# MMOCKING/RIDERS

Measured on AMD Instinct MI355X. Metric: train imgs/sec (RC-Net+SML, 256x512), higher is better.
Workload: dtype bf16; 1 GPU; 2 RC-Net steps (batch 8, K=30, patch 240x100, 256x512) + 1 SML step (batch 16, 256x512) per iteration = 16 images through BOTH stages; each step fwd+loss+bwd+Adam; global_batch=16, parallelism=dp1

## Files before the change

riders_amd/csrc/rd_api.cpp:

```cpp
#include "../../include/riders_hip.h"
#include "rd_kernels.h"
#define rd rd_f16
#include "rd_kernels_decl.h"
#undef rd
#include <math.h>
#include <stdarg.h>
#include <stdio.h>
#include <string.h>
#include <stdlib.h>
#define RD_SLAB_DECL(NS) namespace NS { \
  bool bn_slab_ok(int64_t pixels, int C, int dtype); \
  void launch_bn_bwd_slab(const void* dz, const void* y, const float* mean, const float* rstd, const float* scale, const float* shift, float* dgamma, float* dbeta, \
                          int accumulate, void* dy, int64_t pixels, int C, int act, float slope, int dtype, hipStream_t st); \
  void launch_bn_fwd_slab(const float* stats, int rows, const void* y, const float* gamma, const float* beta, float eps, float momentum, float* running_mean, \
                          float* running_var, float* mean, float* rstd, float* scale, float* shift, void* out, int64_t pixels, int C, int act, float slope, int dtype, \
                          hipStream_t st); \
  const char* bn_slab_kernel_name(int which, int64_t pixels, int dtype, int act); }
RD_SLAB_DECL(rd)
RD_SLAB_DECL(rd_f16)
#undef RD_SLAB_DECL
namespace rd { void launch_augment_vflip_boxes(float* boxes, int B, int K, const float* params, float n_height, hipStream_t st); }
namespace rd { void launch_pack_weights_batch_map(const void* items, int n, const void* map, int blocks, hipStream_t st); }
namespace rd_f16 { void launch_pack_weights_batch_map(const void* items, int n, const void* map, int blocks, hipStream_t st); }

// ... 31 lines not shown
  a.N = d->N; a.Hin = d->Hin; a.Win = d->Win; a.C1 = d->C1; a.C2 = d->C2;
  a.ups = d->upsample ? 1 : 0;
  a.H1 = a.ups ? d->H1 : d->Hin; a.W1 = a.ups ? d->W1 : d->Win;
  a.Cout = d->Cout; a.KH = d->KH; a.KW = d->KW; a.stride = d->stride; a.pad = d->pad; a.dil = d->in_dilate;
  a.OH = d->OH; a.OW = d->OW; a.act = d->act; a.slope = d->slope; a.D1 = d->D1;
  a.scale_h = (float)a.H1 / (float)d->Hin; a.scale_w = (float)a.W1 / (float)d->Win;
  a.M = d->N * d->OH * d->OW;
  a.K = d->KH * d->KW * (d->C1 + d->C2);
  a.Kpad = RD_NS(d->dtype, conv_kpad)(a.K, RD_DT(d->dtype));
  a.pool2 = d->out_reduce2 ? 1 : 0;
  a.d2s = d->out_d2s ? 1 : 0;
  a.s2d = d->in_s2d ? 1 : 0;
}
}

namespace {
struct OptDef { const char* name; int lo, hi; };
const OptDef kOpts[rdt::OPT_COUNT] = {
  {"conv_par", 0, 1}, {"conv3x3_min_blocks", 0, 1 << 30}, {"conv_stem_min_m", 0, 1 << 30}, {"wgrad_blocks", 8, 1 << 16}, {"wgrad_tiny_min_m", 0, 1 << 30},
  {"conv3x3_w8", 0, 1}, {"patch_bn_max", 32, 128}, {"conv3x3_g8", 1, 4096}, {"conv1x1_min_m", 0, 1 << 30}, {"conv_few_min_m", 0, 1 << 30},
  {"frag_v128", 0, 6}, {"frag_v64", 0, 6}, {"frag_v32", 0, 6}, {"frag_split", 0, 1}, {"frag_split_blocks", 0, 1 << 30},
  {"frag32_v128", 0, 3}, {"frag32_v64", 0, 3}, {"frag_lin", 0, 1}, {"conv3x3_frag", 0, 1}, {"bn_gen_ppt", 2, 64}, {"bn_vec_per", 0, 64},
  {"wgrad_tr_tw", 8, 32}, {"frag_db", 0, 1}, {"wgrad_fit", 0, 1}, {"head_np", 256, 1800}, {"head_cpi", 0, 0x888}, {"pw_min_m", 0, 1 << 30}, {"pw_ks", 0, 8}, {"bn_slab", 0, 2},
};
int g_opt_val[rdt::OPT_COUNT];
bool g_opt_set[rdt::OPT_COUNT];
}

extern "C" {

int rd_opt(int id, int dflt) { return (id >= 0 && id < rdt::OPT_COUNT && g_opt_set[id]) ? g_opt_val[id] : dflt; }
int rd_opt_is_set(int id) { return id >= 0 && id < rdt::OPT_COUNT && g_opt_set[id]; }
int rd_set_option(const char* name, int32_t value) {
  if (!name) return fail("set_option: null name");
  for (int i = 0; i < rdt::OPT_COUNT; i++)
    if (!strcmp(name, kOpts[i].name)) {
      g_opt_val[i] = value < kOpts[i].lo ? kOpts[i].lo : (value > kOpts[i].hi ? kOpts[i].hi : value);
      g_opt_set[i] = true;
      return 0;
    }
  return fail("set_option: unknown option '%s'", name);
}
int rd_clear_options(void) { for (int i = 0; i < rdt::OPT_COUNT; i++) g_opt_set[i] = false; return 0; }
int rd_clear_option(const char* name) {
  if (!name) return rd_clear_options();
  for (int i = 0; i < rdt::OPT_COUNT; i++) if (!strcmp(name, kOpts[i].name)) { g_opt_set[i] = false; return 0; }
// ... 999 lines not shown
```

riders_amd/csrc/rd_dwconv.hip:

```cpp
#include "rd_common.h"
#include "rd_kernels.h"

namespace rd {

static unsigned ew_grid(int64_t n) { return (unsigned)std::max<int64_t>(1, std::min<int64_t>(cdiv(n, 256), 4096)); }

template <typename T>
__global__ __launch_bounds__(256) void dwconv_fwd_kernel(const T* __restrict__ x, const float* __restrict__ w, T* __restrict__ y,
                                                         int N, int H, int W, int C, int OH, int OW, int k, int s, int p) {
  const int64_t total = (int64_t)N * OH * OW * C;
  for (int64_t i = (int64_t)blockIdx.x * blockDim.x + threadIdx.x; i < total; i += (int64_t)gridDim.x * blockDim.x) {
    int c = (int)(i % C); int64_t q = i / C;
    int ow = (int)(q % OW); q /= OW; int oh = (int)(q % OH); int n = (int)(q / OH);
    float acc = 0.f;
    for (int kh = 0; kh < k; kh++) {
      int ih = oh * s - p + kh;
      if ((unsigned)ih >= (unsigned)H) continue;
      for (int kw = 0; kw < k; kw++) {
        int iw = ow * s - p + kw;
        if ((unsigned)iw >= (unsigned)W) continue;
        acc += Elem<T>::ld(x + (((int64_t)n * H + ih) * W + iw) * C + c) * w[(c * k + kh) * k + kw];
      }
    }
    Elem<T>::st(y + i, acc);
// ... 50 lines not shown
          acc[j] += g * Elem<T>::ld(x + (((int64_t)n * H + ih) * W + iw) * C + c);
      }
    }
  }
  for (int j = 0; j < k * k; j++) {
    float v = 0.f;
#pragma unroll
    for (int jj = 0; jj < KK; jj++) if (jj == j) v = acc[jj];
    red[t] = v;
    __syncthreads();
    if (pl == 0 && c < C) {
      float sacc = 0.f;
      for (int q = 0; q < PL; q++) sacc += red[q * CB + cl];
      partial[((int64_t)blockIdx.x * C + c) * (k * k) + j] = sacc;
    }
    __syncthreads();
  }
}


#ifndef RD_DW_ST_MODE
#define RD_DW_ST_MODE 1
#endif
static constexpr int DWR = 4;

static constexpr int DW_QMAX = 64;
template <int K> struct DwLds { static constexpr int STR = K == 5 ? 108 : 4 * K * K; };
template <int K>
__device__ __forceinline__ void dw_stage_weights(const float* __restrict__ w, int c0, int nq, float* lds, int cl, bool active,
                                                 float (&wr)[K * K][4]) {
  constexpr int QF = 4 * K * K, STR = DwLds<K>::STR;
  const float* src = w + (int64_t)c0 * K * K;
  if ((reinterpret_cast<uintptr_t>(src) & 15) == 0) {
    for (int i = threadIdx.x; i < nq * (QF / 4); i += blockDim.x) {
      const float4 v = reinterpret_cast<const float4*>(src)[i];
      const int qd = (i * 4) / QF, off = i * 4 - qd * QF;
      *reinterpret_cast<float4*>(lds + qd * STR + off) = v;
    }
  } else {
    for (int i = threadIdx.x; i < nq * QF; i += blockDim.x) { const int qd = i / QF; lds[qd * STR + i - qd * QF] = src[i]; }
  }
  __syncthreads();
  if (active) {
#pragma unroll
    for (int j = 0; j < K * K; j++)
#pragma unroll
      for (int e = 0; e < 4; e++) wr[j][e] = lds[cl * STR + e * K * K + j];
  }
}

template <typename T, int K, int S, int MODE, bool ST>
__global__ __launch_bounds__(256) RD_WAVES_PER_EU((ST && S == 1) ? 2 : 1) void dw_run_kernel(const T* __restrict__ src, const float* __restrict__ w, T* __restrict__ dst, int N,
                                                     int H, int W, int C, int OH, int OW, int p, int QB, int PL, int PPB,
                                                     float* __restrict__ stats) {
  __shared__ __attribute__((aligned(16))) float wl[DW_QMAX * DwLds<K>::STR];
  const int t = threadIdx.x, pl = t / QB, cl = t - pl * QB;
  const int c = (blockIdx.y * QB + cl) * 4;
  const bool active = pl < PL && c < C;
  float wr[K * K][4];
  dw_stage_weights<K>(w, blockIdx.y * QB * 4, min(QB, C / 4 - (int)blockIdx.y * QB), wl, cl, active, wr);
  if (!ST && !active) return;
  float* red = wl;
  if (ST) {
    __syncthreads();
#pragma unroll
    for (int e = 0; e < 8; e++) red[t * 8 + e] = 0.f;
  }
  constexpr int WIN = (DWR - 1) * S + K;
  const int DH = MODE ? H : OH, DW = MODE ? W : OW;
  const int SH = MODE ? OH : H, SW = MODE ? OW : W;
  const int runs = (DW + DWR - 1) / DWR;
  const int64_t M = (int64_t)N * DH * runs;
// ... 39 lines not shown
#pragma unroll
      for (int r = 0; r < DWR; r++)
        if (dw0 + r < DW) {
#pragma unroll
          for (int e = 0; e < 4; e++) { const float v = Elem<T>::rnd(acc[r][e]); u1[e] += v; u2[e] += v * v; }
        }
#pragma unroll
      for (int e = 0; e < 4; e++) { red[t * 8 + e] += u1[e]; red[t * 8 + 4 + e] += u2[e]; }
    }
  }
  if (ST) {
    __syncthreads();
#if RD_DW_ST_MODE == 0
    if (active && pl == 0) {
#pragma unroll
      for (int e = 0; e < 4; e++) {
        float a = 0.f, b = 0.f;
        for (int q = 0; q < PL; q++) { a += red[(q * QB + cl) * 8 + e]; b += red[(q * QB + cl) * 8 + 4 + e]; }
        stats[((int64_t)blockIdx.x * C + c + e) * 2] = a;
        stats[((int64_t)blockIdx.x * C + c + e) * 2 + 1] = b;
      }
    }
#elif RD_DW_ST_MODE == 1
    if (active) {
      for (int e8 = pl; e8 < 8; e8 += PL) {
        float a = 0.f;
        for (int q0 = 0; q0 < PL; q0 += 4) {
          float v[4];
#pragma unroll
          for (int u = 0; u < 4; u++) v[u] = red[(min(q0 + u, PL - 1) * QB + cl) * 8 + e8];
#pragma unroll
          for (int u = 0; u < 4; u++) if (q0 + u < PL) a += v[u];
        }
        stats[((int64_t)blockIdx.x * C + c + (e8 & 3)) * 2 + (e8 >> 2)] = a;
      }
    }
#else
    if (active && pl == 0 && red[t * 8] == 12345.f) stats[0] = 1.f;
#endif
  }
}

template <typename T, int K, int PP, int PH>
__device__ __forceinline__ void dw_dgrad2_rows(const T* __restrict__ dy, const float (&wr)[K * K][4], int n, int dh, int p, int OH, int OW, int C,
                                               int c, const int* coff, const bool* cok, float (&acc)[DWR][4]) {
  constexpr int NJ = (K + 2 - PP) / 2 + 1;
#pragma unroll
  for (int kh = PH; kh < K; kh += 2) {
    const int oh = (dh + p - kh) >> 1;
    const bool rok = (unsigned)oh < (unsigned)OH;
    const T* row = dy + (((int64_t)n * OH + (oh < 0 ? 0 : (oh >= OH ? OH - 1 : oh))) * OW) * C + c;
    float v[NJ][4];
#pragma unroll
    for (int j = 0; j < NJ; j++) ld4z(row + coff[j], rok && cok[j], v[j]);
#pragma unroll
    for (int r = 0; r < DWR; r++)
#pragma unroll
      for (int j = 0; j < NJ; j++) {
        const int kw = r + (K - 1 - PP) - 2 * j;
// ... 72 lines not shown
#pragma unroll
      for (int j = 0; j < WIN; j++) {
        const int iw = cbase + j;
        cok[j] = (unsigned)iw < (unsigned)W;
        coff[j] = (iw < 0 ? 0 : (iw >= W ? W - 1 : iw)) * C;
      }
#pragma unroll
      for (int kh = 0; kh < K; kh++) {
        const int ih = oh * S - p + kh;
        const bool rok = (unsigned)ih < (unsigned)H;
        const T* row = x + (((int64_t)n * H + (ih < 0 ? 0 : (ih >= H ? H - 1 : ih))) * W) * C + c;
        float v[WIN][4];
#pragma unroll
        for (int j = 0; j < WIN; j++) ld4z(row + coff[j], rok && cok[j], v[j]);
#pragma unroll
        for (int kw = 0; kw < K; kw++)
#pragma unroll
          for (int r = 0; r < DWR; r++)
#pragma unroll
            for (int e = 0; e < 4; e++) acc[kh * K + kw][e] = fmaf(g[r][e], v[r * S + kw][e], acc[kh * K + kw][e]);
      }
    }
  }
#pragma unroll
  for (int kh = 0; kh < K; kh++) {
#pragma unroll
    for (int kw = 0; kw < K; kw++)
#pragma unroll
      for (int e = 0; e < 4; e++) red[t][kw][e] = acc[kh * K + kw][e];
    __syncthreads();
    if (cv) {
      for (int kw = pl; kw < K; kw += PL) {
        float s4[4] = {0.f, 0.f, 0.f, 0.f};
        for (int q0 = 0; q0 < PL; q0 += 4) {
          float4 v[4];
#pragma unroll
          for (int u = 0; u < 4; u++) v[u] = *reinterpret_cast<const float4*>(&red[min(q0 + u, PL - 1) * QB + cl][kw][0]);
#pragma unroll
          for (int u = 0; u < 4; u++)
            if (q0 + u < PL) { s4[0] += v[u].x; s4[1] += v[u].y; s4[2] += v[u].z; s4[3] += v[u].w; }
        }
        st4(partial + ((int64_t)blockIdx.x * (K * K) + kh * K + kw) * C + c, s4);
      }
    }
    __syncthreads();
  }
}

__global__ __launch_bounds__(256) void dw_wgrad_finalize_tc_kernel(const float* __restrict__ partial, int rows, int C, int KK, float* dw,
                                                                   int accumulate) {
  __shared__ double red[4][64];
  const int e = threadIdx.x & 63, rg = threadIdx.x >> 6;
  const int i = blockIdx.x * 64 + e, CK = C * KK;
  double a = 0.0;
  if (i < CK)
    for (int r = rg; r < rows; r += 4) a += partial[(int64_t)r * CK + i];
  red[rg][e] = a;
  __syncthreads();
  if (rg == 0 && i < CK) {
    a = red[0][e] + red[1][e] + red[2][e] + red[3][e];
    const int j = i / C, c = i - j * C;
    const int o = c * KK + j;
    dw[o] = accumulate ? dw[o] + (float)a : (float)a;
  }
}

__global__ __launch_bounds__(64) void dwconv_wgrad_finalize_kernel(const float* __restrict__ partial, int rows, int CK, float* dw,
                                                                   int accumulate) {
  const int i = blockIdx.x, lane = threadIdx.x;
// ... 93 lines not shown
  for (int64_t i = (int64_t)blockIdx.x * blockDim.x + threadIdx.x; i < n; i += (int64_t)gridDim.x * blockDim.x) {
    float sc = 1.f + Elem<T>::ld(out + i);
    float p = d[i] * (sc > 0.f ? sc : 0.f);
    bool clamped = (hi > 0.f && p > hi);
    if (!clamped && lo > 0.f && p < lo) clamped = true;
    Elem<T>::st(dout + i, (sc > 0.f && !clamped) ? dpred[i] * d[i] : 0.f);
  }
}
__global__ __launch_bounds__(256) void reciprocal_kernel(const float* __restrict__ x, const float* __restrict__ dy, float* __restrict__ out,
                                                         int64_t n) {
  for (int64_t i = (int64_t)blockIdx.x * blockDim.x + threadIdx.x; i < n; i += (int64_t)gridDim.x * blockDim.x) {
    float v = x[i];
    out[i] = dy ? -dy[i] / (v * v) : 1.f / v;
  }
}

struct RG { int CB, PL, nchunk; };
static RG rgeom(int C) { RG g; int cb = 1; while (cb < C && cb < 256) cb <<= 1; g.CB = cb; g.PL = 256 / cb; g.nchunk = (int)cdiv(C, cb); return g; }
int dw_rows(int64_t pixels, int C) {
  RG g = rgeom(C);
  return (int)std::max<int64_t>(1, std::min<int64_t>(cdiv(pixels, (int64_t)g.PL * 64), 512));
}

struct QG { int QB, PL, nchunk; };
static QG qgeom(int C, int qmax) {
  const int c4 = C / 4;
  QG best = {1, 256, c4}; double bu = -1.0;
  for (int nc = 1; nc <= 256; nc++) {
    const int qb = (int)cdiv(c4, nc);
    if (qb > qmax) continue;
    const int pl = 256 / qb;
    const double u = (double)c4 * pl / (256.0 * nc);
    if (u > bu + 1e-9) { bu = u; best = {qb, pl, nc}; }
  }
  return best;
}
static int dw_upt(int64_t units, const QG& g) {
  (void)units; (void)g;
  return 1;
}
static int dw_stats_ppb(int64_t units, const QG& g) {
  const int64_t upt = std::max<int64_t>(dw_upt(units, g), cdiv(units, (int64_t)g.PL * 1024));
  return (int)(g.PL * upt);
}
template <typename T, int MODE>
static void launch_dw_quad(const void* src, const float* w, void* dst, int N, int H, int W, int C, int OH, int OW, int k, int s, int p, hipStream_t st,
                           float* stats = nullptr) {
  const QG g = qgeom(C, DW_QMAX);
  const int DH = MODE ? H : OH, DW = MODE ? W : OW;
  const int64_t units = (int64_t)N * DH * cdiv(DW, DWR);
  const int ppb = stats ? dw_stats_ppb(units, g) : g.PL * dw_upt(units, g);
  const dim3 grid((unsigned)cdiv(units, ppb), g.nchunk);
#define RD_DWQ(KERNEL) hipLaunchKernelGGL(KERNEL, grid, dim3(256), 0, st, (const T*)src, w, (T*)dst, N, H, W, C, OH, OW, p, g.QB, g.PL, ppb, stats)
#define RD_DWQ2(KERNEL) hipLaunchKernelGGL(KERNEL, grid, dim3(256), 0, st, (const T*)src, w, (T*)dst, N, H, W, C, OH, OW, p, g.QB, g.PL, ppb)
  if (MODE == 0 && stats) {
    if (s == 1) { if (k == 3) RD_DWQ((dw_run_kernel<T, 3, 1, 0, true>)); else RD_DWQ((dw_run_kernel<T, 5, 1, 0, true>)); }
    else { if (k == 3) RD_DWQ((dw_run_kernel<T, 3, 2, 0, true>)); else RD_DWQ((dw_run_kernel<T, 5, 2, 0, true>)); }
  } else if (MODE == 0) {
    if (s == 1) { if (k == 3) RD_DWQ((dw_run_kernel<T, 3, 1, 0, false>)); else RD_DWQ((dw_run_kernel<T, 5, 1, 0, false>)); }
    else { if (k == 3) RD_DWQ((dw_run_kernel<T, 3, 2, 0, false>)); else RD_DWQ((dw_run_kernel<T, 5, 2, 0, false>)); }
  } else if (s == 1) {
    if (k == 3) RD_DWQ((dw_run_kernel<T, 3, 1, 1, false>)); else RD_DWQ((dw_run_kernel<T, 5, 1, 1, false>));
  } else if (p & 1) {
    if (k == 3) RD_DWQ2((dw_dgrad2_kernel<T, 3, 1>)); else RD_DWQ2((dw_dgrad2_kernel<T, 5, 1>));
  } else {
    if (k == 3) RD_DWQ2((dw_dgrad2_kernel<T, 3, 0>)); else RD_DWQ2((dw_dgrad2_kernel<T, 5, 0>));
  }
#undef RD_DWQ
#undef RD_DWQ2
}
static bool dw_quad_ok(int C, int k, int s) { return C % 4 == 0 && (k == 3 || k == 5) && (s == 1 || s == 2); }

int dwconv_stats_rows(int N, int OH, int OW, int C, int k, int s) {
  if (!dw_quad_ok(C, k, s)) return 0;
  const QG g = qgeom(C, DW_QMAX);
  const int64_t units = (int64_t)N * OH * cdiv(OW, DWR);
  return (int)cdiv(units, dw_stats_ppb(units, g));
}
void launch_dwconv_fwd(const void* x, const float* w, void* y, int N, int H, int W, int C, int OH, int OW, int k, int s, int p, int dtype,
                       hipStream_t st, float* stats) {
  if (dw_quad_ok(C, k, s)) {
    if (dtype == 0) launch_dw_quad<float, 0>(x, w, y, N, H, W, C, OH, OW, k, s, p, st, stats);
    else launch_dw_quad<bf16_t, 0>(x, w, y, N, H, W, C, OH, OW, k, s, p, st, stats);
    return;
  }
  int64_t n = (int64_t)N * OH * OW * C;
  if (dtype == 0) hipLaunchKernelGGL((dwconv_fwd_kernel<float>), dim3(ew_grid(n)), dim3(256), 0, st, (const float*)x, w, (float*)y, N, H, W, C, OH, OW, k, s, p);
  else hipLaunchKernelGGL((dwconv_fwd_kernel<bf16_t>), dim3(ew_grid(n)), dim3(256), 0, st, (const bf16_t*)x, w, (bf16_t*)y, N, H, W, C, OH, OW, k, s, p);
}
void launch_dwconv_dgrad(const void* dy, const float* w, void* dx, int N, int H, int W, int C, int OH, int OW, int k, int s, int p,
                         int dtype, hipStream_t st) {
  if (dw_quad_ok(C, k, s)) {
    if (dtype == 0) launch_dw_quad<float, 1>(dy, w, dx, N, H, W, C, OH, OW, k, s, p, st);
    else launch_dw_quad<bf16_t, 1>(dy, w, dx, N, H, W, C, OH, OW, k, s, p, st);
    return;
  }
  int64_t n = (int64_t)N * H * W * C;
  if (dtype == 0) hipLaunchKernelGGL((dwconv_dgrad_kernel<float>), dim3(ew_grid(n)), dim3(256), 0, st, (const float*)dy, w, (float*)dx, N, H, W, C, OH, OW, k, s, p);
  else hipLaunchKernelGGL((dwconv_dgrad_kernel<bf16_t>), dim3(ew_grid(n)), dim3(256), 0, st, (const bf16_t*)dy, w, (bf16_t*)dx, N, H, W, C, OH, OW, k, s, p);
}
struct DwWgradBatch { DwWgradItem it[DW_WGRAD_BATCH_MAX]; };
__global__ __launch_bounds__(256) void dw_wgrad_finalize_batch_kernel(DwWgradBatch b) {
  __shared__ double red[4][64];
  const DwWgradItem it = b.it[blockIdx.y];
  const int e = threadIdx.x & 63, rg = threadIdx.x >> 6;
  const int CK = it.C * it.KK;
  for (int base = blockIdx.x * 64; base < CK; base += gridDim.x * 64) {
    const int i = base + e;
    double a = 0.0;
    if (i < CK) {
      for (int r = rg; r < it.rows; r += 32) {
        float v[8];
#pragma unroll
        for (int q = 0; q < 8; q++) { const int rq = r + 4 * q; const float x = it.partial[(int64_t)(rq < it.rows ? rq : 0) * CK + i]; v[q] = rq < it.rows ? x : 0.f; }
#pragma unroll
// ... 6 lines not shown
      a = red[0][e] + red[1][e] + red[2][e] + red[3][e];
      const int j = i / it.C, c = i - j * it.C;
      const int o = c * it.KK + j;
      it.dw[o] = it.accumulate ? it.dw[o] + (float)a : (float)a;
    }
    __syncthreads();
  }
}
void launch_dw_wgrad_finalize_batch(const DwWgradItem* items, int n, hipStream_t st) {
  for (int base = 0; base < n; base += DW_WGRAD_BATCH_MAX) {
    const int m = std::min(DW_WGRAD_BATCH_MAX, n - base);
    DwWgradBatch b;
    int maxg = 1;
    for (int i = 0; i < m; i++) { b.it[i] = items[base + i]; maxg = std::max(maxg, (int)cdiv(b.it[i].C * b.it[i].KK, 64)); }
    for (int i = m; i < DW_WGRAD_BATCH_MAX; i++) b.it[i] = b.it[0];
    hipLaunchKernelGGL(dw_wgrad_finalize_batch_kernel, dim3((unsigned)std::min(maxg, 1024), (unsigned)m), dim3(256), 0, st, b);
  }
}
void launch_dwconv_wgrad(const void* x, const void* dy, float* partial, float* dw, int accumulate, int N, int H, int W, int C, int OH,
                         int OW, int k, int s, int p, int dtype, hipStream_t st, DwWgradItem* item) {
  if (item) { item->partial = partial; item->dw = dw; item->rows = 0; item->C = C; item->KK = k * k; item->accumulate = accumulate; }
  const int rows = dw_rows((int64_t)N * OH * OW, C);
  if (dw_quad_ok(C, k, s)) {
    const QG g = qgeom(C, 256);
    const int64_t units = (int64_t)N * OH * cdiv(OW, DWR);
    int64_t gx = std::min<int64_t>(512 / g.nchunk, cdiv(units, (int64_t)g.PL * 3));
    gx = std::min<int64_t>(gx, std::max<int64_t>(64, (int64_t)N * OH * OW / 32));
    gx = std::max<int64_t>(1, std::min<int64_t>(gx, rows));
    const dim3 grid((unsigned)gx, g.nchunk);
#define RD_DWG(T, K, S) hipLaunchKernelGGL((dw_wgrad_run_kernel<T, K, S>), grid, dim3(256), 0, st, (const T*)x, (const T*)dy, partial, N, H, W, C, OH, OW, p, g.QB, g.PL)
    if (dtype == 0) {
      if (s == 1) { if (k == 3) RD_DWG(float, 3, 1); else RD_DWG(float, 5, 1); }
      else { if (k == 3) RD_DWG(float, 3, 2); else RD_DWG(float, 5, 2); }
    } else {
      if (s == 1) { if (k == 3) RD_DWG(bf16_t, 3, 1); else RD_DWG(bf16_t, 5, 1); }
      else { if (k == 3) RD_DWG(bf16_t, 3, 2); else RD_DWG(bf16_t, 5, 2); }
    }
#undef RD_DWG
    if (item) { item->rows = (int)gx; return; }
    hipLaunchKernelGGL(dw_wgrad_finalize_tc_kernel, dim3((unsigned)cdiv(C * k * k, 64)), dim3(256), 0, st, partial, (int)gx, C, k * k, dw, accumulate);
    return;
  }
  RG g = rgeom(C);
  dim3 grid(rows, g.nchunk);
#define RD_DW(T, KK) hipLaunchKernelGGL((dwconv_wgrad_kernel<T, KK>), grid, dim3(256), 0, st, (const T*)x, (const T*)dy, partial, N, H, W, C, OH, OW, k, s, p, g.CB, g.PL)
  if (dtype == 0) { if (k <= 3) RD_DW(float, 9); else RD_DW(float, 25); }
  else { if (k <= 3) RD_DW(bf16_t, 9); else RD_DW(bf16_t, 25); }
#undef RD_DW
  hipLaunchKernelGGL(dwconv_wgrad_finalize_kernel, dim3(C * k * k), dim3(64), 0, st, partial, rows, C * k * k, dw, accumulate);
}
void launch_bn_stats(const void* y, float* partial, int64_t pixels, int C, int dtype, hipStream_t st) {
  RG g = rgeom(C);
  dim3 grid(dw_rows(pixels, C), g.nchunk);
  if (dtype == 0) hipLaunchKernelGGL((bn_stats_kernel<float>), grid, dim3(256), 0, st, (const float*)y, partial, pixels, C, g.CB, g.PL);
  else hipLaunchKernelGGL((bn_stats_kernel<bf16_t>), grid, dim3(256), 0, st, (const bf16_t*)y, partial, pixels, C, g.CB, g.PL);
}
template <typename T>
__global__ __launch_bounds__(256) void bilinear_fwd_vec_kernel(const T* __restrict__ x, T* __restrict__ y, int N, int H, int W, int C, int OH,
                                                               int OW, int align) {
  constexpr int VE = Elem<T>::VE;
  const int CV = C / VE;
// ... 126 lines not shown
```

riders_amd/csrc/rd_types.h:

```cpp
#pragma once
#include <hip/hip_runtime.h>
#include <stdint.h>

namespace rdt {

struct ConvArgs {
  const void* src1; const void* src2; const void* w; const float* bias;
  void* dst1; void* dst2; float* stats;
  int N, Hin, Win, C1, C2, H1, W1, Cout, KH, KW, stride, pad, dil, OH, OW, act, D1;
  float slope, scale_h, scale_w;
  int M, K, Kpad, ups;
  int s2d;
  int d2s;
  int pool2;
  const void* add1;
  const float* in_scale; const float* in_shift; int in_act; float in_slope;
  const void* bn_y; const float *bn_scale, *bn_shift, *bn_mean, *bn_rstd; int bn_act; float bn_slope;
};

struct WgradArgs {
  const void* src1; const void* src2; const void* dy; float* slab;
  int N, Hin, Win, C1, C2, H1, W1, Cout, KH, KW, stride, pad, OH, OW;
  float scale_h, scale_w;
  int M, K, ups, nsplit, rows_per_split;
// ... 10 lines not shown

struct LnGradItem { const float* partial[4]; float* dgamma; float* dbeta; int rows[4]; int C, nparts, accumulate, reserved; };
static const int LN_GRAD_BATCH_MAX = 32;
struct DwWgradItem { const float* partial; float* dw; int rows, C, KK, accumulate; };
static const int DW_WGRAD_BATCH_MAX = 64;
struct ColsumItem { const float* partial; float* out; int rows, C, accumulate, reserved; };
static const int COLSUM_BATCH_MAX = 64;

static const int LWG_MAX_ITEMS = 64, LWG_MAX_REDS = 96;

struct LoftrW { const void *wq, *wk, *wv, *wm, *w0, *w2; const float *g1, *b1, *g2, *b2; };

struct LoftrSaved { void *q, *k, *v, *att, *mpre, *msg, *hid, *m2pre; float* stats; };

struct LoftrGrads {
  const void* dout; void *dm2pre, *dhid, *dmpre, *datt, *dq, *dk, *dv, *dx, *dsrc;
  float *lnp1, *lnp2, *dg1, *db1, *dg2, *db2; int accumulate, defer_ln;
  int dsrc_accumulate, reserved;
};

enum RdOpt {
  OPT_CONV_PAR, OPT_CONV3X3_MIN_BLOCKS, OPT_CONV_STEM_MIN_M, OPT_WGRAD_BLOCKS, OPT_WGRAD_TINY_MIN_M, OPT_CONV3X3_W8, OPT_PATCH_BN_MAX,
  OPT_CONV3X3_G8, OPT_CONV1X1_MIN_M, OPT_CONV_FEW_MIN_M, OPT_FRAG_V128, OPT_FRAG_V64, OPT_FRAG_V32, OPT_FRAG_SPLIT, OPT_FRAG_SPLIT_BLOCKS,
  OPT_FRAG32_V128, OPT_FRAG32_V64, OPT_FRAG_LIN, OPT_CONV3X3_FRAG, OPT_BN_GEN_PPT, OPT_BN_VEC_PER, OPT_WGRAD_TR_TW, OPT_FRAG_DB, OPT_WGRAD_FIT, OPT_HEAD_NP, OPT_HEAD_CPI, OPT_PW_MIN_M, OPT_PW_KS, OPT_BN_SLAB, OPT_COUNT
};

}

extern "C" int rd_opt(int id, int dflt);
extern "C" int rd_opt_is_set(int id);
```

Before: 618.6 imgs/s.

## Add column-strip depthwise conv kernels with rolling row window reuse

Adds new depthwise conv kernels where each thread walks down a strip of R output rows over a CW-wide column run. A rolling register window of input rows is reused across all K kernel rows, and the next row is prefetched while the current one is computed. The default mode (dw_col=1) routes forward and dgrad for stride-1 3x3/5x5 convs through the new path when the launch gives enough blocks. Weight-gradient and stats-fused variants are only used in mode 2. The aim is to cut redundant input loads versus the per-row quad kernel, at the cost of higher register pressure and fewer parallel work units.

```diff
diff --git a/riders_amd/csrc/rd_api.cpp b/riders_amd/csrc/rd_api.cpp
--- a/riders_amd/csrc/rd_api.cpp
+++ b/riders_amd/csrc/rd_api.cpp
@@ -77,6 +77,7 @@
   {"frag_v128", 0, 6}, {"frag_v64", 0, 6}, {"frag_v32", 0, 6}, {"frag_split", 0, 1}, {"frag_split_blocks", 0, 1 << 30},
   {"frag32_v128", 0, 3}, {"frag32_v64", 0, 3}, {"frag_lin", 0, 1}, {"conv3x3_frag", 0, 1}, {"bn_gen_ppt", 2, 64}, {"bn_vec_per", 0, 64},
   {"wgrad_tr_tw", 8, 32}, {"frag_db", 0, 1}, {"wgrad_fit", 0, 1}, {"head_np", 256, 1800}, {"head_cpi", 0, 0x888}, {"pw_min_m", 0, 1 << 30}, {"pw_ks", 0, 8}, {"bn_slab", 0, 2},
+  {"dw_col", 0, 2}, {"dw_col_rows", 0, 1024},
 };
 int g_opt_val[rdt::OPT_COUNT];
 bool g_opt_set[rdt::OPT_COUNT];
diff --git a/riders_amd/csrc/rd_dwconv.hip b/riders_amd/csrc/rd_dwconv.hip
--- a/riders_amd/csrc/rd_dwconv.hip
+++ b/riders_amd/csrc/rd_dwconv.hip
@@ -1,5 +1,4 @@
-#include "rd_common.h"
-#include "rd_kernels.h"
+#include "rd_dwconv_common.h"
 
 namespace rd {
 
@@ -96,32 +95,6 @@
 #ifndef RD_DW_ST_MODE
 #define RD_DW_ST_MODE 1
 #endif
-static constexpr int DWR = 4;
-
-static constexpr int DW_QMAX = 64;
-template <int K> struct DwLds { static constexpr int STR = K == 5 ? 108 : 4 * K * K; };
-template <int K>
-__device__ __forceinline__ void dw_stage_weights(const float* __restrict__ w, int c0, int nq, float* lds, int cl, bool active,
-                                                 float (&wr)[K * K][4]) {
-  constexpr int QF = 4 * K * K, STR = DwLds<K>::STR;
-  const float* src = w + (int64_t)c0 * K * K;
-  if ((reinterpret_cast<uintptr_t>(src) & 15) == 0) {
-    for (int i = threadIdx.x; i < nq * (QF / 4); i += blockDim.x) {
-      const float4 v = reinterpret_cast<const float4*>(src)[i];
-      const int qd = (i * 4) / QF, off = i * 4 - qd * QF;
-      *reinterpret_cast<float4*>(lds + qd * STR + off) = v;
-    }
-  } else {
-    for (int i = threadIdx.x; i < nq * QF; i += blockDim.x) { const int qd = i / QF; lds[qd * STR + i - qd * QF] = src[i]; }
-  }
-  __syncthreads();
-  if (active) {
-#pragma unroll
-    for (int j = 0; j < K * K; j++)
-#pragma unroll
-      for (int e = 0; e < 4; e++) wr[j][e] = lds[cl * STR + e * K * K + j];
-  }
-}
 
 template <typename T, int K, int S, int MODE, bool ST>
 __global__ __launch_bounds__(256) RD_WAVES_PER_EU((ST && S == 1) ? 2 : 1) void dw_run_kernel(const T* __restrict__ src, const float* __restrict__ w, T* __restrict__ dst, int N,
@@ -207,19 +180,7 @@
       }
     }
 #elif RD_DW_ST_MODE == 1
-    if (active) {
-      for (int e8 = pl; e8 < 8; e8 += PL) {
-        float a = 0.f;
-        for (int q0 = 0; q0 < PL; q0 += 4) {
-          float v[4];
-#pragma unroll
-          for (int u = 0; u < 4; u++) v[u] = red[(min(q0 + u, PL - 1) * QB + cl) * 8 + e8];
-#pragma unroll
-          for (int u = 0; u < 4; u++) if (q0 + u < PL) a += v[u];
-        }
-        stats[((int64_t)blockIdx.x * C + c + (e8 & 3)) * 2 + (e8 >> 2)] = a;
-      }
-    }
+    if (active) dw_stats_epilogue(red, stats, C, c, QB, PL, pl, cl);
 #else
     if (active && pl == 0 && red[t * 8] == 12345.f) stats[0] = 1.f;
 #endif
@@ -338,29 +299,7 @@
       }
     }
   }
-#pragma unroll
-  for (int kh = 0; kh < K; kh++) {
-#pragma unroll
-    for (int kw = 0; kw < K; kw++)
-#pragma unroll
-      for (int e = 0; e < 4; e++) red[t][kw][e] = acc[kh * K + kw][e];
-    __syncthreads();
-    if (cv) {
-      for (int kw = pl; kw < K; kw += PL) {
-        float s4[4] = {0.f, 0.f, 0.f, 0.f};
-        for (int q0 = 0; q0 < PL; q0 += 4) {
-          float4 v[4];
-#pragma unroll
-          for (int u = 0; u < 4; u++) v[u] = *reinterpret_cast<const float4*>(&red[min(q0 + u, PL - 1) * QB + cl][kw][0]);
-#pragma unroll
-          for (int u = 0; u < 4; u++)
-            if (q0 + u < PL) { s4[0] += v[u].x; s4[1] += v[u].y; s4[2] += v[u].z; s4[3] += v[u].w; }
-        }
-        st4(partial + ((int64_t)blockIdx.x * (K * K) + kh * K + kw) * C + c, s4);
-      }
-    }
-    __syncthreads();
-  }
+  dw_wgrad_epilogue<K>(acc, red, partial, C, c, cv, QB, PL, pl, cl);
 }
 
 __global__ __launch_bounds__(256) void dw_wgrad_finalize_tc_kernel(const float* __restrict__ partial, int rows, int C, int KK, float* dw,
@@ -500,19 +439,6 @@
   return (int)std::max<int64_t>(1, std::min<int64_t>(cdiv(pixels, (int64_t)g.PL * 64), 512));
 }
 
-struct QG { int QB, PL, nchunk; };
-static QG qgeom(int C, int qmax) {
-  const int c4 = C / 4;
-  QG best = {1, 256, c4}; double bu = -1.0;
-  for (int nc = 1; nc <= 256; nc++) {
-    const int qb = (int)cdiv(c4, nc);
-    if (qb > qmax) continue;
-    const int pl = 256 / qb;
-    const double u = (double)c4 * pl / (256.0 * nc);
-    if (u > bu + 1e-9) { bu = u; best = {qb, pl, nc}; }
-  }
-  return best;
-}
 static int dw_upt(int64_t units, const QG& g) {
   (void)units; (void)g;
   return 1;
@@ -551,6 +477,7 @@
 
 int dwconv_stats_rows(int N, int OH, int OW, int C, int k, int s) {
   if (!dw_quad_ok(C, k, s)) return 0;
+  if (const int R = dw_col_rows(3, N, OH, OW, C, k, s)) return dw_col_stats_rows(N, OH, OW, C, k, R);
   const QG g = qgeom(C, DW_QMAX);
   const int64_t units = (int64_t)N * OH * cdiv(OW, DWR);
   return (int)cdiv(units, dw_stats_ppb(units, g));
@@ -558,6 +485,7 @@
 void launch_dwconv_fwd(const void* x, const float* w, void* y, int N, int H, int W, int C, int OH, int OW, int k, int s, int p, int dtype,
                        hipStream_t st, float* stats) {
   if (dw_quad_ok(C, k, s)) {
+    if (const int R = dw_col_rows(stats ? 3 : 0, N, OH, OW, C, k, s)) { launch_dw_col(0, x, w, y, N, H, W, C, OH, OW, k, p, R, dtype, st, stats); return; }
     if (dtype == 0) launch_dw_quad<float, 0>(x, w, y, N, H, W, C, OH, OW, k, s, p, st, stats);
     else launch_dw_quad<bf16_t, 0>(x, w, y, N, H, W, C, OH, OW, k, s, p, st, stats);
     return;
@@ -569,6 +497,7 @@
 void launch_dwconv_dgrad(const void* dy, const float* w, void* dx, int N, int H, int W, int C, int OH, int OW, int k, int s, int p,
                          int dtype, hipStream_t st) {
   if (dw_quad_ok(C, k, s)) {
+    if (const int R = dw_col_rows(1, N, OH, OW, C, k, s)) { launch_dw_col(1, dy, w, dx, N, H, W, C, OH, OW, k, p, R, dtype, st, nullptr); return; }
     if (dtype == 0) launch_dw_quad<float, 1>(dy, w, dx, N, H, W, C, OH, OW, k, s, p, st);
     else launch_dw_quad<bf16_t, 1>(dy, w, dx, N, H, W, C, OH, OW, k, s, p, st);
     return;
@@ -621,21 +550,26 @@
   if (item) { item->partial = partial; item->dw = dw; item->rows = 0; item->C = C; item->KK = k * k; item->accumulate = accumulate; }
   const int rows = dw_rows((int64_t)N * OH * OW, C);
   if (dw_quad_ok(C, k, s)) {
-    const QG g = qgeom(C, 256);
-    const int64_t units = (int64_t)N * OH * cdiv(OW, DWR);
-    int64_t gx = std::min<int64_t>(512 / g.nchunk, cdiv(units, (int64_t)g.PL * 3));
-    gx = std::min<int64_t>(gx, std::max<int64_t>(64, (int64_t)N * OH * OW / 32));
-    gx = std::max<int64_t>(1, std::min<int64_t>(gx, rows));
-    const dim3 grid((unsigned)gx, g.nchunk);
+    int64_t gx;
+    if (const int R = dw_col_rows(2, N, OH, OW, C, k, s)) {
+      gx = launch_dw_wgrad_col(x, dy, partial, N, H, W, C, OH, OW, k, p, R, rows, dtype, st);
+    } else {
+      const QG g = qgeom(C, 256);
+      const int64_t units = (int64_t)N * OH * cdiv(OW, DWR);
+      gx = std::min<int64_t>(512 / g.nchunk, cdiv(units, (int64_t)g.PL * 3));
+      gx = std::min<int64_t>(gx, std::max<int64_t>(64, (int64_t)N * OH * OW / 32));
+      gx = std::max<int64_t>(1, std::min<int64_t>(gx, rows));
+      const dim3 grid((unsigned)gx, g.nchunk);
 #define RD_DWG(T, K, S) hipLaunchKernelGGL((dw_wgrad_run_kernel<T, K, S>), grid, dim3(256), 0, st, (const T*)x, (const T*)dy, partial, N, H, W, C, OH, OW, p, g.QB, g.PL)
-    if (dtype == 0) {
-      if (s == 1) { if (k == 3) RD_DWG(float, 3, 1); else RD_DWG(float, 5, 1); }
-      else { if (k == 3) RD_DWG(float, 3, 2); else RD_DWG(float, 5, 2); }
-    } else {
-      if (s == 1) { if (k == 3) RD_DWG(bf16_t, 3, 1); else RD_DWG(bf16_t, 5, 1); }
-      else { if (k == 3) RD_DWG(bf16_t, 3, 2); else RD_DWG(bf16_t, 5, 2); }
-    }
+      if (dtype == 0) {
+        if (s == 1) { if (k == 3) RD_DWG(float, 3, 1); else RD_DWG(float, 5, 1); }
+        else { if (k == 3) RD_DWG(float, 3, 2); else RD_DWG(float, 5, 2); }
+      } else {
+        if (s == 1) { if (k == 3) RD_DWG(bf16_t, 3, 1); else RD_DWG(bf16_t, 5, 1); }
+        else { if (k == 3) RD_DWG(bf16_t, 3, 2); else RD_DWG(bf16_t, 5, 2); }
+      }
 #undef RD_DWG
+    }
     if (item) { item->rows = (int)gx; return; }
     hipLaunchKernelGGL(dw_wgrad_finalize_tc_kernel, dim3((unsigned)cdiv(C * k * k, 64)), dim3(256), 0, st, partial, (int)gx, C, k * k, dw, accumulate);
     return;
diff --git a/riders_amd/csrc/rd_dwconv_col.hip b/riders_amd/csrc/rd_dwconv_col.hip
--- /dev/null
+++ b/riders_amd/csrc/rd_dwconv_col.hip
@@ -0,0 +1,292 @@
+#include "rd_dwconv_common.h"
+
+namespace rd {
+
+template <typename T> struct DwRaw;
+template <> struct DwRaw<float> { typedef float4 type; };
+template <> struct DwRaw<bf16_t> { typedef uint2 type; };
+__device__ __forceinline__ void ld4raw(const float* p, float4& r) { r = *reinterpret_cast<const float4*>(p); }
+__device__ __forceinline__ void ld4raw(const bf16_t* p, uint2& r) { r = *reinterpret_cast<const uint2*>(p); }
+__device__ __forceinline__ void raw4z(const float4& r, bool ok, float (&o)[4]) {
+  o[0] = ok ? r.x : 0.f; o[1] = ok ? r.y : 0.f; o[2] = ok ? r.z : 0.f; o[3] = ok ? r.w : 0.f;
+}
+__device__ __forceinline__ void raw4z(const uint2& r, bool ok, float (&o)[4]) {
+  const unsigned x = ok ? r.x : 0u, y = ok ? r.y : 0u;
+  o[0] = half_lo_f32(x); o[1] = half_hi_f32(x);
+  o[2] = half_lo_f32(y); o[3] = half_hi_f32(y);
+}
+__device__ __forceinline__ int clampi(int v, int n) { return v < 0 ? 0 : (v >= n ? n - 1 : v); }
+
+template <typename T, int K, int MODE, bool ST, int CW>
+__global__ __launch_bounds__(256) RD_WAVES_PER_EU(1) void dw_col_kernel(const T* __restrict__ src, const float* __restrict__ w, T* __restrict__ dst, int N,
+                                                     int H, int W, int C, int OH, int OW, int p, int QB, int PL, int PPB, int R,
+                                                     float* __restrict__ stats) {
+  __shared__ __attribute__((aligned(16))) float wl[DW_QMAX * DwLds<K>::STR];
+  typedef typename DwRaw<T>::type Raw;
+  const int tid = threadIdx.x, pl = tid / QB, cl = tid - pl * QB;
+  const int c = (blockIdx.y * QB + cl) * 4;
+  const bool active = pl < PL && c < C;
+  float wr[K * K][4];
+  dw_stage_weights<K>(w, blockIdx.y * QB * 4, min(QB, C / 4 - (int)blockIdx.y * QB), wl, cl, active, wr);
+  if (!ST && !active) return;
+  float* red = wl;
+  if (ST) {
+    __syncthreads();
+#pragma unroll
+    for (int e = 0; e < 8; e++) red[tid * 8 + e] = 0.f;
+  }
+  constexpr int WIN = CW - 1 + K;
+  const int DH = MODE ? H : OH, DW = MODE ? W : OW;
+  const int SH = MODE ? OH : H, SW = MODE ? OW : W;
+  const int runs = (DW + CW - 1) / CW, spi = (DH + R - 1) / R;
+  const int64_t M = (int64_t)N * spi * runs;
+  const int64_t mbeg = (int64_t)xcd_contiguous(blockIdx.x, gridDim.x) * PPB, mend = !active ? 0 : (mbeg + PPB < M ? mbeg + PPB : M);
+  const int steps = R + K - 1;
+  for (int64_t m = mbeg + pl; m < mend; m += PL) {
+    const int rw = (int)(m % runs); int64_t q = m / runs; const int sp = (int)(q % spi); const int n = (int)(q / spi);
+    const int dw0 = rw * CW, r0 = sp * R;
+    const int cbase = MODE ? dw0 + p - (K - 1) : dw0 - p;
+    int coff[WIN]; bool cok[WIN];
+#pragma unroll
+    for (int j = 0; j < WIN; j++) {
+      const int sw = cbase + j;
+      cok[j] = (unsigned)sw < (unsigned)SW;
+      coff[j] = clampi(sw, SW) * C;
+    }
+    const T* img = src + (int64_t)n * SH * SW * C + c;
+    T* out = dst + (int64_t)n * DH * DW * C + c;
+    const int sh0 = MODE ? r0 + R - 1 + p : r0 - p;
+    Raw raw[WIN];
+    {
+      const T* row = img + (int64_t)clampi(sh0, SH) * SW * C;
+#pragma unroll
+      for (int j = 0; j < WIN; j++) ld4raw(row + coff[j], raw[j]);
+    }
+    float acc[K][CW][4];
+    for (int t0 = 0; t0 < steps; t0 += K) {
+#pragma unroll
+      for (int tt = 0; tt < K; tt++) {
+        const int t = t0 + tt;
+        if (t < steps) {
+          const int sh = MODE ? sh0 - t : sh0 + t;
+          const bool rok = (unsigned)sh < (unsigned)SH;
+          float v[WIN][4];
+#pragma unroll
+          for (int j = 0; j < WIN; j++) raw4z(raw[j], rok && cok[j], v[j]);
+          {
+            const T* row = img + (int64_t)clampi(MODE ? sh - 1 : sh + 1, SH) * SW * C;
+#pragma unroll
+            for (int j = 0; j < WIN; j++) ld4raw(row + coff[j], raw[j]);
+          }
+          sched_fence();
+#pragma unroll
+          for (int kh = 0; kh < K; kh++) {
+            const int slot = (tt - kh + K) % K;
+            const int jr = t - kh;
+            if (jr >= 0 && jr < R) {
+              if (kh == 0) {
+#pragma unroll
+                for (int r = 0; r < CW; r++)
+#pragma unroll
+                  for (int e = 0; e < 4; e++) acc[slot][r][e] = 0.f;
+              }
+#pragma unroll
+              for (int kw = 0; kw < K; kw++)
+#pragma unroll
+                for (int r = 0; r < CW; r++)
+#pragma unroll
+                  for (int e = 0; e < 4; e++) acc[slot][r][e] = fmaf(v[MODE ? r + K - 1 - kw : r + kw][e], wr[kh * K + kw][e], acc[slot][r][e]);
+              if (kh == K - 1) {
+                const int dh = MODE ? r0 + R - 1 - jr : r0 + jr;
+                if (dh < DH) {
+                  T* orow = out + ((int64_t)dh * DW + dw0) * C;
+#pragma unroll
+                  for (int r = 0; r < CW; r++)
+                    if (dw0 + r < DW) st4(orow + (int64_t)r * C, acc[slot][r]);
+                  if (ST) {
+                    float u1[4] = {0.f, 0.f, 0.f, 0.f}, u2[4] = {0.f, 0.f, 0.f, 0.f};
+#pragma unroll
+                    for (int r = 0; r < CW; r++)
+                      if (dw0 + r < DW) {
+#pragma unroll
+                        for (int e = 0; e < 4; e++) { const float z = Elem<T>::rnd(acc[slot][r][e]); u1[e] += z; u2[e] += z * z; }
+                      }
+#pragma unroll
+                    for (int e = 0; e < 4; e++) { red[tid * 8 + e] += u1[e]; red[tid * 8 + 4 + e] += u2[e]; }
+                  }
+                }
+              }
+            }
+          }
+        }
+      }
+    }
+  }
+  if (ST) {
+    __syncthreads();
+    if (active) dw_stats_epilogue(red, stats, C, c, QB, PL, pl, cl);
+  }
+}
+
+template <typename T, int K, int CW>
+__global__ __launch_bounds__(256) RD_WAVES_PER_EU(1) void dw_wgrad_col_kernel(const T* __restrict__ x, const T* __restrict__ dy, float* __restrict__ partial,
+                                                           int N, int H, int W, int C, int OH, int OW, int p, int QB, int PL, int R) {
+  __shared__ float red[256][K][4];
+  typedef typename DwRaw<T>::type Raw;
+  const int tid = threadIdx.x, pl = tid / QB, cl = tid - pl * QB;
+  const int c = (blockIdx.y * QB + cl) * 4;
+  const bool cv = pl < PL && c < C;
+  constexpr int WIN = CW - 1 + K;
+  const int runs = (OW + CW - 1) / CW, spi = (H + R - 1) / R;
+  const int64_t units = (int64_t)N * spi * runs;
+  const int64_t per = cdiv(units, gridDim.x);
+  const int64_t ubeg = (int64_t)xcd_contiguous(blockIdx.x, gridDim.x) * per, uend = ubeg + per < units ? ubeg + per : units;
+  float acc[K * K][4];
+#pragma unroll
+  for (int j = 0; j < K * K; j++)
+#pragma unroll
+    for (int e = 0; e < 4; e++) acc[j][e] = 0.f;
+  if (cv) {
+    for (int64_t m = ubeg + pl; m < uend; m += PL) {
+      const int rw = (int)(m % runs); int64_t q = m / runs; const int sp = (int)(q % spi); const int n = (int)(q / spi);
+      const int ow0 = rw * CW, r0 = sp * R;
+      int coff[WIN]; bool cok[WIN];
+#pragma unroll
+      for (int j = 0; j < WIN; j++) {
+        const int iw = ow0 - p + j;
+        cok[j] = (unsigned)iw < (unsigned)W;
+        coff[j] = clampi(iw, W) * C;
+      }
+      int goff[CW]; bool gok[CW];
+#pragma unroll
+      for (int r = 0; r < CW; r++) { gok[r] = ow0 + r < OW; goff[r] = (gok[r] ? ow0 + r : OW - 1) * C; }
+      const T* ximg = x + (int64_t)n * H * W * C + c;
+      const T* gimg = dy + (int64_t)n * OH * OW * C + c;
+      const int oh0 = r0 + p - (K - 1);
+      float g[K][CW][4];
+#pragma unroll
+      for (int d = 0; d < K - 1; d++) {
+        const int oh = oh0 + d;
+        const T* row = gimg + (int64_t)clampi(oh, OH) * OW * C;
+#pragma unroll
+        for (int r = 0; r < CW; r++) ld4z(row + goff[r], (unsigned)oh < (unsigned)OH && gok[r], g[d][r]);
+      }
+      Raw rx[WIN], rg[CW];
+      {
+        const T* row = ximg + (int64_t)clampi(r0, H) * W * C;
+#pragma unroll
+        for (int j = 0; j < WIN; j++) ld4raw(row + coff[j], rx[j]);
+        const T* grow = gimg + (int64_t)clampi(r0 + p, OH) * OW * C;
+#pragma unroll
+        for (int r = 0; r < CW; r++) ld4raw(grow + goff[r], rg[r]);
+      }
+      for (int t0 = 0; t0 < R; t0 += K) {
+#pragma unroll
+        for (int tt = 0; tt < K; tt++) {
+          const int t = t0 + tt;
+          if (t < R) {
+            const int ih = r0 + t, ohn = ih + p;
+            const bool xok = ih < H, nok = (unsigned)ohn < (unsigned)OH;
+            float v[WIN][4];
+#pragma unroll
+            for (int j = 0; j < WIN; j++) raw4z(rx[j], xok && cok[j], v[j]);
+#pragma unroll
+            for (int r = 0; r < CW; r++) raw4z(rg[r], nok && gok[r], g[(tt + K - 1) % K][r]);
+            {
+              const T* row = ximg + (int64_t)clampi(ih + 1, H) * W * C;
+#pragma unroll
+              for (int j = 0; j < WIN; j++) ld4raw(row + coff[j], rx[j]);
+              const T* grow = gimg + (int64_t)clampi(ohn + 1, OH) * OW * C;
+#pragma unroll
+              for (int r = 0; r < CW; r++) ld4raw(grow + goff[r], rg[r]);
+            }
+            sched_fence();
+#pragma unroll
+            for (int kh = 0; kh < K; kh++) {
+              const int slot = (tt + K - 1 - kh) % K;
+#pragma unroll
+              for (int kw = 0; kw < K; kw++)
+#pragma unroll
+                for (int r = 0; r < CW; r++)
+#pragma unroll
+                  for (int e = 0; e < 4; e++) acc[kh * K + kw][e] = fmaf(g[slot][r][e], v[r + kw][e], acc[kh * K + kw][e]);
+            }
+          }
+        }
+      }
+    }
+  }
+  dw_wgrad_epilogue<K>(acc, red, partial, C, c, cv, QB, PL, pl, cl);
+}
+
+static int dw_col_cw(int k) { return k == 5 ? 2 : DWR; }
+static int dw_col_routed_rows(int dir, int N, int OH, int OW, int C, int k) {
+  if (dir == 2 && OH < 16) return 0;
+  const QG g = qgeom(C, dir == 2 ? 256 : DW_QMAX);
+  const int64_t runs = cdiv(OW, dw_col_cw(k)), want = dir == 2 ? 160 : (k == 5 ? 320 : 420);
+  for (int spi = 1; spi <= OH; spi++) {
+    const int R = (int)cdiv(OH, spi);
+    if (R < 3) break;
+    if (spi > 1 && R == (int)cdiv(OH, spi - 1)) continue;
+    const int64_t bx = cdiv((int64_t)N * cdiv(OH, R) * runs, g.PL);
+    if (bx * g.nchunk < want) continue;
+    if (dir == 2 && bx > dw_rows((int64_t)N * OH * OW, C)) return 0;
+    return R;
+  }
+  return 0;
+}
+int dw_col_rows(int dir, int N, int OH, int OW, int C, int k, int s) {
+  const int mode = rd_opt(OPT_DW_COL, 1);
+  if (mode == 0 || C % 4 != 0 || (k != 3 && k != 5) || s != 1 || OH < 1) return 0;
+  if (mode != 2 && (dir == 2 || dir == 3)) return 0;
+  int R = rd_opt(OPT_DW_COL_ROWS, 0);
+  if (R <= 0) R = dw_col_routed_rows(dir == 3 ? 0 : dir, N, OH, OW, C, k);
+  if (R <= 0) {
+    if (mode != 2) return 0;
+    R = k;
+  }
+  return std::min(R, OH);
+}
+static int dw_col_ppb(int64_t units, const QG& g, bool stats) {
+  return (int)(g.PL * (stats ? std::max<int64_t>(1, cdiv(units, (int64_t)g.PL * 1024)) : 1));
+}
+int dw_col_stats_rows(int N, int OH, int OW, int C, int k, int R) {
+  const QG g = qgeom(C, DW_QMAX);
+  const int64_t units = (int64_t)N * cdiv(OH, R) * cdiv(OW, dw_col_cw(k));
+  return (int)cdiv(units, dw_col_ppb(units, g, true));
+}
+template <typename T>
+static void launch_dw_col_t(int mode, const void* src, const float* w, void* dst, int N, int H, int W, int C, int OH, int OW, int k, int p, int R,
+                            hipStream_t st, float* stats) {
+  const QG g = qgeom(C, DW_QMAX);
+  const int DH = mode ? H : OH, DW = mode ? W : OW;
+  const int64_t units = (int64_t)N * cdiv(DH, R) * cdiv(DW, dw_col_cw(k));
+  const int ppb = dw_col_ppb(units, g, stats != nullptr);
+  const dim3 grid((unsigned)cdiv(units, ppb), g.nchunk);
+#define RD_DWC(K, MODE, ST) hipLaunchKernelGGL((dw_col_kernel<T, K, MODE, ST, (K == 5 ? 2 : DWR)>), grid, dim3(256), 0, st, (const T*)src, w, (T*)dst, N, H, W, C, OH, OW, p, g.QB, g.PL, ppb, R, stats)
+  if (mode == 0 && stats) { if (k == 3) RD_DWC(3, 0, true); else RD_DWC(5, 0, true); }
+  else if (mode == 0) { if (k == 3) RD_DWC(3, 0, false); else RD_DWC(5, 0, false); }
+  else { if (k == 3) RD_DWC(3, 1, false); else RD_DWC(5, 1, false); }
+#undef RD_DWC
+}
+void launch_dw_col(int mode, const void* src, const float* w, void* dst, int N, int H, int W, int C, int OH, int OW, int k, int p, int R, int dtype,
+                   hipStream_t st, float* stats) {
+  if (dtype == 0) launch_dw_col_t<float>(mode, src, w, dst, N, H, W, C, OH, OW, k, p, R, st, stats);
+  else launch_dw_col_t<bf16_t>(mode, src, w, dst, N, H, W, C, OH, OW, k, p, R, st, stats);
+}
+int launch_dw_wgrad_col(const void* x, const void* dy, float* partial, int N, int H, int W, int C, int OH, int OW, int k, int p, int R, int max_rows,
+                        int dtype, hipStream_t st) {
+  const QG g = qgeom(C, 256);
+  const int64_t units = (int64_t)N * cdiv(H, R) * cdiv(OW, dw_col_cw(k));
+  int64_t gx = std::min<int64_t>(std::max(1, 512 / g.nchunk), cdiv(units, g.PL));
+  gx = std::max<int64_t>(1, std::min<int64_t>(gx, max_rows));
+  gx = cdiv(units, cdiv(units, gx));
+  const dim3 grid((unsigned)gx, g.nchunk);
+#define RD_DWGC(T, K) hipLaunchKernelGGL((dw_wgrad_col_kernel<T, K, (K == 5 ? 2 : DWR)>), grid, dim3(256), 0, st, (const T*)x, (const T*)dy, partial, N, H, W, C, OH, OW, p, g.QB, g.PL, R)
+  if (dtype == 0) { if (k == 3) RD_DWGC(float, 3); else RD_DWGC(float, 5); }
+  else { if (k == 3) RD_DWGC(bf16_t, 3); else RD_DWGC(bf16_t, 5); }
+#undef RD_DWGC
+  return (int)gx;
+}
+
+}
diff --git a/riders_amd/csrc/rd_dwconv_common.h b/riders_amd/csrc/rd_dwconv_common.h
--- /dev/null
+++ b/riders_amd/csrc/rd_dwconv_common.h
@@ -0,0 +1,97 @@
+#pragma once
+#include "rd_common.h"
+#include "rd_kernels.h"
+
+namespace rd {
+
+static constexpr int DWR = 4;
+static constexpr int DW_QMAX = 64;
+template <int K> struct DwLds { static constexpr int STR = K == 5 ? 108 : 4 * K * K; };
+template <int K>
+__device__ __forceinline__ void dw_stage_weights(const float* __restrict__ w, int c0, int nq, float* lds, int cl, bool active,
+                                                 float (&wr)[K * K][4]) {
+  constexpr int QF = 4 * K * K, STR = DwLds<K>::STR;
+  const float* src = w + (int64_t)c0 * K * K;
+  if ((reinterpret_cast<uintptr_t>(src) & 15) == 0) {
+    for (int i = threadIdx.x; i < nq * (QF / 4); i += blockDim.x) {
+      const float4 v = reinterpret_cast<const float4*>(src)[i];
+      const int qd = (i * 4) / QF, off = i * 4 - qd * QF;
+      *reinterpret_cast<float4*>(lds + qd * STR + off) = v;
+    }
+  } else {
+    for (int i = threadIdx.x; i < nq * QF; i += blockDim.x) { const int qd = i / QF; lds[qd * STR + i - qd * QF] = src[i]; }
+  }
+  __syncthreads();
+  if (active) {
+#pragma unroll
+    for (int j = 0; j < K * K; j++)
+#pragma unroll
+      for (int e = 0; e < 4; e++) wr[j][e] = lds[cl * STR + e * K * K + j];
+  }
+}
+
+__device__ __forceinline__ void dw_stats_epilogue(const float* red, float* __restrict__ stats, int C, int c, int QB, int PL, int pl, int cl) {
+  for (int e8 = pl; e8 < 8; e8 += PL) {
+    float a = 0.f;
+    for (int q0 = 0; q0 < PL; q0 += 4) {
+      float v[4];
+#pragma unroll
+      for (int u = 0; u < 4; u++) v[u] = red[(min(q0 + u, PL - 1) * QB + cl) * 8 + e8];
+#pragma unroll
+      for (int u = 0; u < 4; u++) if (q0 + u < PL) a += v[u];
+    }
+    stats[((int64_t)blockIdx.x * C + c + (e8 & 3)) * 2 + (e8 >> 2)] = a;
+  }
+}
+
+template <int K>
+__device__ __forceinline__ void dw_wgrad_epilogue(const float (&acc)[K * K][4], float (*red)[K][4], float* __restrict__ partial, int C, int c,
+                                                  bool cv, int QB, int PL, int pl, int cl) {
+  const int t = threadIdx.x;
+#pragma unroll
+  for (int kh = 0; kh < K; kh++) {
+#pragma unroll
+    for (int kw = 0; kw < K; kw++)
+#pragma unroll
+      for (int e = 0; e < 4; e++) red[t][kw][e] = acc[kh * K + kw][e];
+    __syncthreads();
+    if (cv) {
+      for (int kw = pl; kw < K; kw += PL) {
+        float s4[4] = {0.f, 0.f, 0.f, 0.f};
+        for (int q0 = 0; q0 < PL; q0 += 4) {
+          float4 v[4];
+#pragma unroll
+          for (int u = 0; u < 4; u++) v[u] = *reinterpret_cast<const float4*>(&red[min(q0 + u, PL - 1) * QB + cl][kw][0]);
+#pragma unroll
+          for (int u = 0; u < 4; u++)
+            if (q0 + u < PL) { s4[0] += v[u].x; s4[1] += v[u].y; s4[2] += v[u].z; s4[3] += v[u].w; }
+        }
+        st4(partial + ((int64_t)blockIdx.x * (K * K) + kh * K + kw) * C + c, s4);
+      }
+    }
+    __syncthreads();
+  }
+}
+
+struct QG { int QB, PL, nchunk; };
+static inline QG qgeom(int C, int qmax) {
+  const int c4 = C / 4;
+  QG best = {1, 256, c4}; double bu = -1.0;
+  for (int nc = 1; nc <= 256; nc++) {
+    const int qb = (int)cdiv(c4, nc);
+    if (qb > qmax) continue;
+    const int pl = 256 / qb;
+    const double u = (double)c4 * pl / (256.0 * nc);
+    if (u > bu + 1e-9) { bu = u; best = {qb, pl, nc}; }
+  }
+  return best;
+}
+
+int dw_col_rows(int dir, int N, int OH, int OW, int C, int k, int s);
+int dw_col_stats_rows(int N, int OH, int OW, int C, int k, int R);
+void launch_dw_col(int mode, const void* src, const float* w, void* dst, int N, int H, int W, int C, int OH, int OW, int k, int p, int R, int dtype,
+                   hipStream_t st, float* stats);
+int launch_dw_wgrad_col(const void* x, const void* dy, float* partial, int N, int H, int W, int C, int OH, int OW, int k, int p, int R, int max_rows,
+                        int dtype, hipStream_t st);
+
+}
diff --git a/riders_amd/csrc/rd_types.h b/riders_amd/csrc/rd_types.h
--- a/riders_amd/csrc/rd_types.h
+++ b/riders_amd/csrc/rd_types.h
@@ -56,7 +56,7 @@
 enum RdOpt {
   OPT_CONV_PAR, OPT_CONV3X3_MIN_BLOCKS, OPT_CONV_STEM_MIN_M, OPT_WGRAD_BLOCKS, OPT_WGRAD_TINY_MIN_M, OPT_CONV3X3_W8, OPT_PATCH_BN_MAX,
   OPT_CONV3X3_G8, OPT_CONV1X1_MIN_M, OPT_CONV_FEW_MIN_M, OPT_FRAG_V128, OPT_FRAG_V64, OPT_FRAG_V32, OPT_FRAG_SPLIT, OPT_FRAG_SPLIT_BLOCKS,
-  OPT_FRAG32_V128, OPT_FRAG32_V64, OPT_FRAG_LIN, OPT_CONV3X3_FRAG, OPT_BN_GEN_PPT, OPT_BN_VEC_PER, OPT_WGRAD_TR_TW, OPT_FRAG_DB, OPT_WGRAD_FIT, OPT_HEAD_NP, OPT_HEAD_CPI, OPT_PW_MIN_M, OPT_PW_KS, OPT_BN_SLAB, OPT_COUNT
+  OPT_FRAG32_V128, OPT_FRAG32_V64, OPT_FRAG_LIN, OPT_CONV3X3_FRAG, OPT_BN_GEN_PPT, OPT_BN_VEC_PER, OPT_WGRAD_TR_TW, OPT_FRAG_DB, OPT_WGRAD_FIT, OPT_HEAD_NP, OPT_HEAD_CPI, OPT_PW_MIN_M, OPT_PW_KS, OPT_BN_SLAB, OPT_DW_COL, OPT_DW_COL_ROWS, OPT_COUNT
 };
 
 }
```

Result: no change. 620.3 imgs/s, median of 6 (+0.3%).
